# CMU-SAFARI/Scrooge

Hardware: AMD Instinct MI355X
Metric: aligned pairs/s (+ GCUPS) at W=64, 10kb reads; 1/2/4/8 MI355X (higher is better)
Workload: dtype u64

## Files before the change

scrooge_amd/api.py:

```python
import contextlib
import ctypes as C
import os
import subprocess
import sys
from collections import namedtuple

HERE = os.path.dirname(os.path.abspath(__file__))
_LIB = None

Alignment = namedtuple("Alignment", ["cigar", "edit_distance"])

SCRG_OK = 0
SCRG_ERR_INVALID_ARG = 1
SCRG_ERR_BAD_BASE = 2
SCRG_ERR_NO_DEVICE = 3
SCRG_ERR_HIP = 4
SCRG_ERR_OOM = 5
SCRG_ERR_CIGAR_OVERFLOW = 6
SCRG_PAIR_OVER_EDIT_LIMIT = 7
SCRG_PAIR_NOT_BEST = 8
SCRG_OUT_ALL, SCRG_OUT_TEXT, SCRG_OUT_RUNS = 0, 1, 2
SCRG_OUT_BEST = 4
SCRG_OUT_DISTANCE = 16
DEVICE_STATUS_OVER_EDIT_LIMIT = 2
# ... 896 lines not shown
        with self._call_limit(max_edits, max_edit_per_mille):
            self._check(self.lib.scrg_align_device(self.h, C.byref(self._params(kw)), int(n_pairs),
                                                   _ptr(seq), _ptr(pairs), _ptr(runs), _ptr(ed),
                                                   _ptr(n_runs), _ptr(status)))

    def align_device_edits(self, n_pairs, seq, pairs, streams_u8, ed, stream_len, status, n_runs=None, max_edits=None,
                           max_edit_per_mille=None, **kw):
        with self._call_limit(max_edits, max_edit_per_mille):
            self._check(self.lib.scrg_align_device_edits(self.h, C.byref(self._params(kw)), int(n_pairs),
                                                         _ptr(seq), _ptr(pairs), _ptr(streams_u8), _ptr(ed),
                                                         _ptr(stream_len), _ptr(status), _ptr(n_runs)))

    def align_device_distance(self, n_pairs, seq, pairs, ed, text_end, status, max_edits=None, max_edit_per_mille=None, **kw):
        with self._call_limit(max_edits, max_edit_per_mille):
            self._check(_lazy(self.lib, "scrg_align_device_distance")(self.h, C.byref(self._params(kw)), int(n_pairs), _ptr(seq), _ptr(pairs),
                                                                      _ptr(ed), _ptr(text_end), _ptr(status)))

    def diff_lengths(self, kind, n_pairs, seq, pairs, runs, run_offset, run_offset_stride, n_runs, diff_len, **kw):
        ro = C.c_void_p(pairs.data_ptr() + 32) if run_offset is None else _ptr(run_offset)
        self._check(_lazy(self.lib, "scrg_diff_lengths")(self.h, C.byref(self._params(kw)), _diff_kind(kind), int(n_pairs), _ptr(seq), _ptr(pairs),
                                                         _ptr(runs), ro, int(run_offset_stride), _ptr(n_runs), _ptr(diff_len)))

    def diff_render(self, kind, n_pairs, seq, pairs, runs, run_offset, run_offset_stride, n_runs, diff_len, diff_offset, diff_text_u8, bad_i32,
                    capacity=None, **kw):
        ro = C.c_void_p(pairs.data_ptr() + 32) if run_offset is None else _ptr(run_offset)
        cap = int(diff_text_u8.numel()) if capacity is None else int(capacity)
        self._check(_lazy(self.lib, "scrg_diff_render")(self.h, C.byref(self._params(kw)), _diff_kind(kind), int(n_pairs), _ptr(seq), _ptr(pairs),
                                                        _ptr(runs), ro, int(run_offset_stride), _ptr(n_runs), _ptr(diff_len), _ptr(diff_offset),
                                                        _ptr(diff_text_u8), cap, _ptr(bad_i32)))

    def compact_runs(self, n_pairs, pairs, runs, n_runs, dense_off, dense):
        self._check(self.lib.scrg_compact_runs(self.h, int(n_pairs), _ptr(pairs), _ptr(runs),
                                               _ptr(n_runs), _ptr(dense_off), _ptr(dense)))

    def select_best(self, n_pairs, group_key_u32, ed, status, n_runs, is_best_u8=None):
        self._check(_lazy(self.lib, "scrg_select_best")(self.h, int(n_pairs), _ptr(group_key_u32), _ptr(ed), _ptr(status), _ptr(n_runs),
                                                        _ptr(is_best_u8)))

    def compact_runs_packed(self, n_pairs, pairs, runs, n_runs, dense_off, packed_u8, **kw):
        self._check(self.lib.scrg_compact_runs_packed(self.h, C.byref(self._params(kw)), int(n_pairs), _ptr(pairs),
                                                      _ptr(runs), _ptr(n_runs), _ptr(dense_off), _ptr(packed_u8)))

    def unpack_runs(self, n_runs, packed_u8, runs_u8):
        self._check(self.lib.scrg_unpack_runs(self.h, int(n_runs), _ptr(packed_u8), _ptr(runs_u8)))

    def encode_edit_stream(self, n_pairs, pairs, runs, n_runs, stream_u8, stream_off_i64, stream_len_i32, total_i64, **kw):
        self._check(self.lib.scrg_encode_edit_stream(self.h, C.byref(self._params(kw)), int(n_pairs), _ptr(pairs), _ptr(runs), _ptr(n_runs),
                                                     _ptr(stream_u8), int(stream_u8.numel()), _ptr(stream_off_i64),
                                                     _ptr(stream_len_i32), _ptr(total_i64)))

    def decode_edit_stream(self, n_pairs, stream_u8, stream_off_i64, stream_len_i32, read_len_i64, read_len_stride,
                           dense_off_i64, dense_u8, n_runs_i32, bad_i32, **kw):
        self._check(self.lib.scrg_decode_edit_stream(self.h, C.byref(self._params(kw)), int(n_pairs), _ptr(stream_u8),
                                                     int(stream_u8.numel()), _ptr(stream_off_i64), _ptr(stream_len_i32), _ptr(read_len_i64),
                                                     int(read_len_stride),
                                                     _ptr(dense_off_i64) if dense_off_i64 is not None else None,
                                                     _ptr(dense_u8) if dense_u8 is not None else None,
                                                     int(dense_u8.numel() * dense_u8.element_size() // 2) if dense_u8 is not None else 0,
                                                     _ptr(n_runs_i32), _ptr(bad_i32)))

    def ascii_to_twobit(self, count, lens, ascii_off, ascii, twobit_off, twobit, bad):
        self._check(self.lib.scrg_ascii_to_twobit(self.h, int(count), _ptr(lens), _ptr(ascii_off),
                                                  _ptr(ascii), _ptr(twobit_off), _ptr(twobit),
                                                  _ptr(bad)))

    def last_kernel_ms(self):
        ms = C.c_float(0)
        self._check(self.lib.scrg_last_kernel_ms(self.h, C.byref(ms)))
        return float(ms.value)

    def debug_stats(self):
        out = (C.c_uint64 * 12)()
        self._check(self.lib.scrg_debug_stats(self.h, out))
        return {"rounds": int(out[0]), "dc_steps": int(out[1]), "tb_macro_steps": int(out[2]),
                "cycles_fetch": int(out[3]), "cycles_setup": int(out[4]), "cycles_dc": int(out[5]),
                "cycles_tb": int(out[6]), "cycles_tb_loop": int(out[7]), "diag_rounds": int(out[8]),
                "diag_fallbacks": int(out[9]), "cycles_diag_dc": int(out[10]), "cycles_diag_tb": int(out[11])}

    def debug_stats_lane(self):
        out = (C.c_uint64 * 12)()
        self._check(self.lib.scrg_debug_stats(self.h, out))
        o = [int(x) for x in out]
        big = 1 << 62
        return {"rounds": o[0], "short_text_rounds": o[1], "cycles_pass1": o[2], "cycles_fetch": o[3], "cycles_setup": o[4],
                "cycles_table": o[5], "cycles_traceback": o[6], "life_ticks_sum": o[7], "last_start": o[8],
                "first_start": big - o[9], "last_end": o[10], "first_end": big - o[11]}

    def resolved_params(self, **kw):
        out = Params()
        st = self.lib.scrg_params_resolve(C.byref(self._params(kw)), C.byref(out))
        if st != SCRG_OK:
            raise ScroogeError(st, "invalid parameters")
        return out

    def query_launch(self, **kw):
        a, b, c, d = C.c_int32(), C.c_int32(), C.c_int32(), C.c_int32()
        self._check(self.lib.scrg_query_launch(self.h, C.byref(self._params(kw)), C.byref(a),
                                               C.byref(b), C.byref(c), C.byref(d)))
        return {"n_waves": a.value, "pairs_per_wave": b.value, "lds_bytes": c.value,
                "n_cus": d.value}
```

scrooge_amd/csrc/genasm_kernels.h:

```cpp
#pragma once

#include <hip/hip_runtime.h>
#include <stdint.h>

#include <type_traits>

#include "../../include/scrooge_amd.h"

namespace scrg {

constexpr int SPILL_ROWS = 72;

struct AlignArgs {
    const uint64_t* seq;
    const scrg_pair_desc* pairs;
    uint16_t* runs;
    int64_t* ed;
    union {
        uint32_t* n_runs;
        uint32_t* text_end;
    };
    uint32_t* status;
    uint32_t* run_count;
    uint32_t* counter;
    uint32_t* spill;
    uint32_t n_pairs;
    int32_t W;
    int32_t tb_limit;
    int32_t lds_rows;
    uint32_t text_stride;
    uint32_t read_stride;
    uint64_t* stats;
    int32_t debug;
    uint32_t stranded;
    uint32_t max_edits;
    uint32_t per_mille;
    uint32_t text_rev;
};
enum LaneOutput : int { LANE_OUT_RUNS = 0, LANE_OUT_EDITS = 1, LANE_OUT_NONE = 2 };
template <typename F> inline void with_lane_output(LaneOutput out, F&& f)
{
    if (out == LANE_OUT_NONE) f(std::integral_constant<int, LANE_OUT_NONE>{});
    else if (out == LANE_OUT_EDITS) f(std::integral_constant<int, LANE_OUT_EDITS>{});
    else f(std::integral_constant<int, LANE_OUT_RUNS>{});
}
enum LaneStatus : uint32_t { LANE_STATUS_DONE = 0, LANE_STATUS_OVERFLOW = 1, LANE_STATUS_OVER_EDIT_LIMIT = 2, LANE_STATUS_NOT_BEST = 3 };

#if defined(SCRG_ABLATE) && !defined(SCRG_STATS)
#define SCRG_STATS 1
#endif
#if defined(SCRG_STATS) && !defined(SCRG_SELECT)
#define SCRG_SELECT 1
#endif
constexpr int32_t SCRG_SWITCH_NO_DIAG = 32;
constexpr int32_t SCRG_SWITCH_MW_TABLE = 256;
constexpr int32_t SCRG_SWITCH_SPLIT = 512;
constexpr int32_t SCRG_SWITCH_NO_SPLIT = 1024;
constexpr int32_t SCRG_SAFE_SWITCHES = SCRG_SWITCH_NO_DIAG | SCRG_SWITCH_MW_TABLE | SCRG_SWITCH_SPLIT | SCRG_SWITCH_NO_SPLIT;
#ifdef SCRG_SELECT
#define SCRG_SEL(flags, bit) (((flags) & (bit)) != 0)
constexpr bool SCRG_HAVE_SELECT = true;
#else
#define SCRG_SEL(flags, bit) false
constexpr bool SCRG_HAVE_SELECT = false;
#endif
#ifdef SCRG_STATS
#define SCRG_TIMING(args) ((args).stats != nullptr)
#define SCRG_SW(args, bit) (((args).debug & (bit)) != 0)
constexpr bool SCRG_HAVE_STATS = true;
#else
#define SCRG_TIMING(args) false
#define SCRG_SW(args, bit) false
constexpr bool SCRG_HAVE_STATS = false;
#endif
#ifdef SCRG_ABLATE
#define SCRG_ABL(args, bit) (((args).debug & (bit)) != 0)
constexpr int32_t SCRG_ALLOWED_SWITCHES = 0x1ff | SCRG_SAFE_SWITCHES;
#elif defined(SCRG_STATS)
#define SCRG_ABL(args, bit) false
constexpr int32_t SCRG_ALLOWED_SWITCHES = SCRG_SAFE_SWITCHES | 1 | 64 | 128;
#elif defined(SCRG_SELECT)
#define SCRG_ABL(args, bit) false
constexpr int32_t SCRG_ALLOWED_SWITCHES = SCRG_SAFE_SWITCHES;
#else
#define SCRG_ABL(args, bit) false
constexpr int32_t SCRG_ALLOWED_SWITCHES = 0;
#endif

#ifdef __HIPCC__
#define SCRG_HD __host__ __device__
#else
#define SCRG_HD
#endif

hipError_t launch_align(int lanes_per_pair, const AlignArgs& a, int grid, size_t lds_bytes, hipStream_t s);
hipError_t launch_align_multiword(int lanes_per_pair, const AlignArgs& a, int grid, size_t lds_bytes, hipStream_t s);
hipError_t launch_align_lane(const AlignArgs& a, int grid, size_t lds_bytes, hipStream_t s, LaneOutput out = LANE_OUT_RUNS);
SCRG_HD inline unsigned lane_lds_bytes(LaneOutput out = LANE_OUT_RUNS) { return 64u * ((out == LANE_OUT_NONE ? 0u : 68u + 36u) + 32u + 8u); }
hipError_t launch_align_lane_split(const AlignArgs& a, int grid, hipStream_t s);
constexpr int LANE_SPLIT_PRODUCERS_PER_CU = 8;

SCRG_HD inline unsigned lane_mw_len_bytes(int tb_limit) { return (((unsigned)tb_limit + 3u) & ~3u) + 4u; }
SCRG_HD inline unsigned lane_mw_lds_bytes(int tb_limit, LaneOutput out = LANE_OUT_RUNS) { return out == LANE_OUT_NONE ? 0u : 64u * (68u + lane_mw_len_bytes(tb_limit)); }
SCRG_HD inline size_t lane_mw_table_bytes(int tb_limit) { return (size_t)tb_limit * 2u * ((unsigned)tb_limit / 64u + 1u) * 64u * 8u; }
hipError_t launch_align_lane_mw(const AlignArgs& a, int grid, size_t lds_bytes, hipStream_t s, LaneOutput out = LANE_OUT_RUNS);
SCRG_HD inline bool lane_wide_serves(int W, int tb_limit) { return W <= 128 && tb_limit >= 32 && tb_limit <= 63; }
SCRG_HD inline unsigned lane_wide_lds_bytes(int W, LaneOutput out = LANE_OUT_RUNS) { return 64u * ((out == LANE_OUT_NONE ? 0u : 68u + 36u) + (W <= 64 ? 40u : 80u)); }
hipError_t launch_align_lane_wide(const AlignArgs& a, int grid, size_t lds_bytes, hipStream_t s, LaneOutput out = LANE_OUT_RUNS);
SCRG_HD inline bool lane_parts_serves(int W, int tb_limit)
{
    return W > 64 && W <= 256 && ((tb_limit >= 64 && tb_limit <= 127) || (W > 128 && tb_limit >= 1 && tb_limit <= 63));
}
SCRG_HD inline unsigned lane_parts_lds_bytes(int W, LaneOutput out = LANE_OUT_RUNS)
{
    const unsigned nw = ((unsigned)W + 63u) / 64u, slot = nw == 2u ? 16u : 32u;
    return 64u * ((out == LANE_OUT_NONE ? 0u : 68u + 20u) + 5u * slot + 16u * nw);
}
SCRG_HD inline size_t lane_parts_checkpoint_bytes(int W) { return (size_t)8u * 4u * (((unsigned)W + 63u) / 64u) * 64u * 4u; }
hipError_t launch_align_lane_parts(const AlignArgs& a, int grid, size_t lds_bytes, hipStream_t s, LaneOutput out = LANE_OUT_RUNS);

SCRG_HD inline unsigned stored_row_dwords(int W, int tb_limit)
{
    if (W <= 64) return tb_limit > 31 ? 128u : 32u;
    const unsigned sw = (unsigned)tb_limit / 64u + 1u;
    return 64u * sw * sw * 2u;
}

constexpr unsigned DIAG_WIDE_ROWS = 8;
constexpr unsigned DIAG_LATE_BASE = 128;
constexpr unsigned DIAG_PARK_DWORD = 392;
constexpr unsigned DIAG_SLOT_DWORDS = DIAG_PARK_DWORD + 4 + 1;
SCRG_HD inline unsigned slot_stride_dwords(int W, int tb_limit, int lanes_per_pair, int lds_rows)
{
    unsigned s = (unsigned)lds_rows * stored_row_dwords(W, tb_limit) + 1u;
    if (W == 64 && lanes_per_pair == 8 && tb_limit <= 31 && s < DIAG_SLOT_DWORDS) s = DIAG_SLOT_DWORDS;
    return s;
}

enum AlignForm : int {
    FORM_ROWS,
    FORM_ROWS_MW,
// ... 72 lines not shown
```

scrooge_amd/csrc/genasm_lane_kernel.hip:

```cpp

#include <hip/hip_runtime.h>
#include <stdint.h>
#include <type_traits>

#include "lane_common.h"

namespace scrg {

constexpr int LANE_TB_COLS = 31;
constexpr uint32_t LANE_RING_BYTES = 68;
constexpr uint32_t LANE_SCRATCH_BYTES = 36;
constexpr uint32_t LANE_EQ_BYTES = 32;
constexpr uint32_t LANE_NOMATCH_BYTES = 8;
constexpr uint32_t LANE_WAVE_LDS_BYTES = 64u * (LANE_RING_BYTES + LANE_SCRATCH_BYTES + LANE_EQ_BYTES + LANE_NOMATCH_BYTES);
constexpr uint32_t LANE_EQ_SLOT_STRIDE = 512;
constexpr uint32_t LANE_EQ_REGION_BYTES = 4u * LANE_EQ_SLOT_STRIDE;
constexpr uint32_t LANE_EQ_FIELD_MASK = 3u * LANE_EQ_SLOT_STRIDE;
constexpr uint32_t LANE_REST_BYTES = LANE_WAVE_LDS_BYTES - LANE_EQ_REGION_BYTES;
constexpr int LANE_EQ_AHEAD = 8;

__device__ __forceinline__ uint32_t lane_read_offset(uint32_t fwd_offset, uint32_t read_idx, uint32_t read_len, uint32_t revm)
{
    return bitop3<TT_BFI>(sub_sat_u32(read_len - read_idx, 64u), fwd_offset, revm);
}
__device__ __forceinline__ void lane_pattern_rev(const Planes pw, uint32_t left, uint32_t revm, bool any_rev, uint64_t& rlo, uint64_t& rhi)
{
    rlo = brev64(pw.lo);
    rhi = brev64(pw.hi);
    if (any_rev) {
        const uint32_t sh = sub_sat_u32(64u, left);
        const uint64_t flo = ~(pw.lo << sh), fhi = ~(pw.hi << sh);
        rlo = ((uint64_t)bitop3<TT_BFI>((uint32_t)(flo >> 32), (uint32_t)(rlo >> 32), revm) << 32) | bitop3<TT_BFI>((uint32_t)flo, (uint32_t)rlo, revm);
        rhi = ((uint64_t)bitop3<TT_BFI>((uint32_t)(fhi >> 32), (uint32_t)(rhi >> 32), revm) << 32) | bitop3<TT_BFI>((uint32_t)fhi, (uint32_t)rhi, revm);
    }
}

constexpr uint32_t LANE_TEXT_REV = 1u << 7;
__device__ __forceinline__ uint32_t lane_text_offset(uint32_t ref_idx, uint32_t text_len, uint32_t tr_in)
{
    return bitop3<TT_BFI>(text_rev_at(text_len, ref_idx, 0u).at, ref_idx, neg_mask(tr_in << 24));
}
__device__ __forceinline__ void lane_text_rev(Planes& tw, uint32_t text_len, uint32_t ref_idx, uint32_t tr_in)
{
    const uint32_t tm = neg_mask(tr_in << 24);
    const uint32_t sh = text_rev_at(text_len, ref_idx, 0u).sh;
    const uint64_t flo = ~brev64(tw.lo << sh), fhi = ~brev64(tw.hi << sh);
    tw.lo = ((uint64_t)bitop3<TT_BFI>((uint32_t)(flo >> 32), (uint32_t)(tw.lo >> 32), tm) << 32) | bitop3<TT_BFI>((uint32_t)flo, (uint32_t)tw.lo, tm);
    tw.hi = ((uint64_t)bitop3<TT_BFI>((uint32_t)(fhi >> 32), (uint32_t)(tw.hi >> 32), tm) << 32) | bitop3<TT_BFI>((uint32_t)fhi, (uint32_t)tw.hi, tm);
}

template <bool SHORT_N>
__device__ __forceinline__ void lane_window_table(const Planes tw, const uint64_t rlo, const uint64_t rhi, const uint32_t n, const uint32_t m,
                                                  const uint32_t stop, uint64_t (&tab)[LANE_TB_COLS],
                                                  const uint32_t eq_b, const uint32_t nomatch_b)
{
    const uint64_t valid = ~0ull << (64u - m);
    const uint32_t rl0 = (uint32_t)rlo, rl1 = (uint32_t)(rlo >> 32), rh0 = (uint32_t)rhi, rh1 = (uint32_t)(rhi >> 32);
    const uint32_t iv0 = ~(uint32_t)valid, iv1 = ~(uint32_t)(valid >> 32);
    {
        lds_write64(eq_b, make_uint2(~(rl0 | rh0) | iv0, ~(rl1 | rh1) | iv1));
        lds_write64(eq_b + LANE_EQ_SLOT_STRIDE, make_uint2((rl0 & ~rh0) | iv0, (rl1 & ~rh1) | iv1));
        lds_write64(eq_b + 2u * LANE_EQ_SLOT_STRIDE, make_uint2((~rl0 & rh0) | iv0, (~rl1 & rh1) | iv1));
        lds_write64(eq_b + 3u * LANE_EQ_SLOT_STRIDE, make_uint2((rl0 & rh0) | iv0, (rl1 & rh1) | iv1));
        if (SHORT_N) lds_write64(nomatch_b, make_uint2(iv0, iv1));
    }
    const uint32_t tl0 = (uint32_t)tw.lo, tl1 = (uint32_t)(tw.lo >> 32), th0 = (uint32_t)tw.hi, th1 = (uint32_t)(tw.hi >> 32);
    const uint32_t xe0 = bitop3<TT_BFI>(tl0, th0 << 1, 0x55555555u), xo0 = bitop3<TT_BFI>(th0, tl0 >> 1, 0xaaaaaaaau);
    const uint32_t xe1 = bitop3<TT_BFI>(tl1, th1 << 1, 0x55555555u), xo1 = bitop3<TT_BFI>(th1, tl1 >> 1, 0xaaaaaaaau);
    auto eq_addr = [&](int i) -> uint32_t {
        const int b = i & 31;
        const uint32_t x = (b & 1) ? (i < 32 ? xo0 : xo1) : (i < 32 ? xe0 : xe1);
        const int f = (b & 1) ? b - 1 : b;
        const uint32_t u = f >= 9 ? x >> (f - 9) : x << (9 - f);
        const uint32_t a = bitop3<TT_ANDOR>(u, LANE_EQ_FIELD_MASK, eq_b);
        if (!SHORT_N) return a;
        return bitop3<TT_BFI>(a, nomatch_b, neg_mask((uint32_t)i - n));
    };
    uint2 eqw[LANE_EQ_AHEAD];
#pragma unroll
    for (int k = 0; k < LANE_EQ_AHEAD; k++) eqw[k] = lds_read64(eq_addr(63 - k));
    uint32_t pv0 = (uint32_t)valid, pv1 = (uint32_t)(valid >> 32), mv0 = 0u, mv1 = 0u;
#pragma unroll
    for (int i = 63; i >= 0; i--) {
        const uint2 eq_now = eqw[(63 - i) % LANE_EQ_AHEAD];
        if (i - LANE_EQ_AHEAD >= 0) eqw[(63 - i) % LANE_EQ_AHEAD] = lds_read64(eq_addr(i - LANE_EQ_AHEAD));
        {
            const uint32_t eq0 = eq_now.x, eq1 = eq_now.y;
            const uint32_t xv0 = eq0 | mv0, xv1 = eq1 | mv1;
            const uint32_t t0 = eq0 & pv0, t1 = eq1 & pv1;
            const uint64_t sum = add64(((uint64_t)t1 << 32) | t0, ((uint64_t)pv1 << 32) | pv0);
            const uint32_t xh0 = bitop3<TT_XH>((uint32_t)sum, pv0, eq0), xh1 = bitop3<TT_XH>((uint32_t)(sum >> 32), pv1, eq1);
            const uint32_t ph0 = bitop3<TT_PH>(mv0, xh0, pv0), ph1 = bitop3<TT_PH>(mv1, xh1, pv1);
            const uint32_t mh0 = pv0 & xh0, mh1 = pv1 & xh1;
            const uint64_t phs = shl1(((uint64_t)ph1 << 32) | ph0);
            const uint64_t mhs = shl1(((uint64_t)mh1 << 32) | mh0);
            pv0 = bitop3<TT_PVN>((uint32_t)mhs, xv0, (uint32_t)phs);
            pv1 = bitop3<TT_PVN>((uint32_t)(mhs >> 32), xv1, (uint32_t)(phs >> 32));
            mv0 = (uint32_t)phs & xv0;
            mv1 = (uint32_t)(phs >> 32) & xv1;
            if (i < LANE_TB_COLS)
                tab[i] = ((uint64_t)bitop3<TT_NOR3>(pv1, ph1, stop) << 32) | bitop3<TT_V0>(pv1, ph1, xh1);
        }
    }
}

template <int OUT>
__global__ __launch_bounds__(256, 4) void genasm_lane_kernel(AlignArgs a)
{
    constexpr bool EDITS = OUT == LANE_OUT_EDITS, NONE = OUT == LANE_OUT_NONE;
    constexpr uint32_t REST_BYTES = NONE ? 64u * LANE_NOMATCH_BYTES : LANE_REST_BYTES;
    constexpr uint32_t STAGE_BYTES = NONE ? 0u : 64u * (LANE_RING_BYTES + LANE_SCRATCH_BYTES);
    extern __shared__ __attribute__((aligned(16))) uint32_t lds[];
    char* const lds_b = reinterpret_cast<char*>(lds);

    const uint32_t lane = threadIdx.x & 63u;
    const uint32_t wave = threadIdx.x >> 6, wpg = blockDim.x >> 6;
    const uint32_t wave_b = wpg * LANE_EQ_REGION_BYTES + wave * REST_BYTES;
    const uint32_t ring_b = wave_b + lane * LANE_RING_BYTES;
    const uint32_t scr_b = wave_b + 64u * LANE_RING_BYTES + lane * LANE_SCRATCH_BYTES;
    uint8_t* const lds8 = reinterpret_cast<uint8_t*>(lds);
    const uint32_t lds0 = (uint32_t)(uintptr_t)(__attribute__((address_space(3))) char*)lds_b;
    const uint32_t eq_b = lds0 + wave * LANE_EQ_REGION_BYTES + lane * 8u;
    const uint32_t nomatch_b = lds0 + wave_b + STAGE_BYTES + lane * LANE_NOMATCH_BYTES;
    const uint32_t W = (uint32_t)a.W;
    const uint32_t TBL = (uint32_t)a.tb_limit;

    bool has_pair = false;
    uint32_t pair = 0;
    const uint64_t* text_w = a.seq;
    const uint64_t* read_w = a.seq;
    uint32_t tr_in = 0;
    uint64_t cigar_off = 0;
    uint32_t text_len = 0, read_len = 0, cigar_cap = 0;
    uint32_t ref_idx = 0, read_idx = 0, edits = 0;
    uint32_t lim = 0xffffffffu;
    uint32_t revm = 0;
    int32_t nr = -1;
    uint32_t flushed = 0;
    uint32_t pos = 0;
    uint32_t mbase = 0;
    WindowWords twords = {0, 0, 0, 0}, pwords = {0, 0, 0, 0};
    bool queue_empty = false;
    const bool timing = SCRG_TIMING(a);
    uint64_t cy_fetch = 0, cy_setup = 0, cy_dc = 0, cy_tb = 0, cy_p1 = 0;
    uint32_t st_rounds = 0, st_gen = 0;
    const uint64_t rt0 = timing ? __builtin_amdgcn_s_memrealtime() : 0;

    auto write_piece = [&]() {
        if constexpr (!NONE) scrg::write_piece<EDITS>(a, lds, ring_b, cigar_off, cigar_cap, flushed, !SCRG_ABL(a, 16));
    };
    auto flush_pieces = [&]() {
        if constexpr (!NONE) {
            const bool need = has_pair && (EDITS ? pos - flushed >= 32u : nr - (int32_t)flushed >= 15);
            if (__any(need)) {
                if (need) write_piece();
            }
        }
    };
    auto ring_guard = [&](uint32_t fill, uint32_t limit) {
        if (__any(has_pair && fill >= limit)) {
            if (has_pair && fill >= (EDITS ? 32u : 16u)) write_piece();
        }
    };

    uint32_t rot = hw_wave_slot();
    for (;;) {
        if (!SCRG_SW(a, 1)) rotate_priority(rot++);
        const uint64_t tm0 = timing ? __builtin_readcyclecounter() : 0;
        for (;;) {
            const bool over = has_pair && edits > lim;
            const bool fin = over || (has_pair && read_idx >= read_len);
            if (__any(fin)) {
                if (over) abandon_pair<OUT>(a, pair, edits);
                else if constexpr (NONE) { if (fin) retire_pair_distance(a, pair, edits, ref_idx); }
                else if (fin) retire_pair<EDITS>(a, lds, ring_b, pair, cigar_off, cigar_cap, flushed, EDITS ? pos : (uint32_t)(nr + 1), nr, edits, !SCRG_ABL(a, 16));
                has_pair = has_pair && !fin;
            }
            const bool want = !has_pair && !queue_empty;
            if (!__any(want)) break;
            const uint32_t idx = claim_pairs(a, lane, want);
            const bool got = want && idx < a.n_pairs;
            if (__any(want && idx >= a.n_pairs)) queue_empty = true;
            if (got) {
                const scrg_pair_desc pd = a.pairs[idx];
                pair = idx;
                const TextStretch ts = text_stretch(pd.text_off, pd.text_len, a.text_rev != 0u, a.text_stride);
                text_w = a.seq + (ts.off >> 5);
                const uint64_t r_off = a.stranded ? pd.read_off & ~SCRG_READ_REVCOMP : pd.read_off;
                revm = (a.stranded && (pd.read_off & SCRG_READ_REVCOMP)) ? 0xffffffffu : 0u;
                read_w = a.seq + (r_off >> 5);
                tr_in = ((uint32_t)ts.off & 31u) | (((uint32_t)r_off & 31u) << 8) | (ts.rev ? LANE_TEXT_REV : 0u);
                text_len = ts.len;
                read_len = (uint32_t)pd.read_len;
                lim = pair_edit_limit(a, read_len);
                if constexpr (NONE) {
                    ref_idx = read_idx = edits = 0;
                } else {
                    cigar_off = pd.cigar_off;
                    cigar_cap = pd.cigar_cap > 0xffffffffull ? 0xffffffffu : (uint32_t)pd.cigar_cap;
                    ref_idx = read_idx = edits = flushed = pos = mbase = 0;
                    nr = -1;
                }
                has_pair = true;
                twords = load_window_words_at(text_w, tr_in & 31u, ts.rev ? text_rev_at(text_len, 0u, 0u).at : 0u, a.text_stride);
                pwords = load_window_words_at(read_w, tr_in >> 8, lane_read_offset(0u, 0u, read_len, revm), a.read_stride);
            }
        }
        if (!__any(has_pair)) break;
        const bool wave_rev = a.stranded && __any(has_pair && revm != 0u);
        const bool wave_trev = a.text_rev && __any(has_pair && (tr_in & LANE_TEXT_REV) != 0u);

        const uint64_t tm1 = timing ? __builtin_readcyclecounter() : 0;
        const uint32_t n = has_pair ? min(W, sub_sat_u32(text_len, ref_idx)) : 0u;
        const uint32_t m = has_pair ? min(W, read_len - read_idx) : 1u;
        Planes tw = window_planes(twords);
        const Planes pw = window_planes(pwords);
        if (wave_trev) lane_text_rev(tw, text_len, ref_idx, tr_in);
        asm volatile("" :: "v"(tw.lo), "v"(tw.hi), "v"(pw.lo), "v"(pw.hi) : "memory");
        flush_pieces();
        const uint64_t tm2 = timing ? __builtin_readcyclecounter() : 0;

        uint64_t tab[LANE_TB_COLS];
        const uint32_t jlim = has_pair ? min(m, TBL) : 0u;
        const uint32_t stop = 0x80000000u >> jlim;
        const bool short_n = __any(has_pair && n != 64u);
        uint64_t rlo, rhi;
        lane_pattern_rev(pw, read_len - read_idx, revm, wave_rev, rlo, rhi);
        if (SCRG_ABL(a, 2)) {
#pragma unroll
            for (int i = 0; i < LANE_TB_COLS; i++) tab[i] = ((uint64_t)~stop << 32) | (((uint32_t)tw.lo * (uint32_t)(i + 1)) | stop);
        } else if (short_n) {
            lane_window_table<true>(tw, rlo, rhi, n, m, stop, tab, eq_b, nomatch_b);
            st_gen++;
        } else {
            lane_window_table<false>(tw, rlo, rhi, n, m, stop, tab, eq_b, nomatch_b);
        }
        const uint64_t tm3 = timing ? __builtin_readcyclecounter() : 0;

        {
            uint32_t j = 0, ti, nDm = 0, Xm = 0, nIm = 0;
            auto walk = [&](auto full_tag) {
                constexpr bool FULL = decltype(full_tag)::value;
#pragma unroll
                for (int i = 0; i < LANE_TB_COLS; i++) {
                    if (!FULL && (uint32_t)i >= TBL) continue;
                    const uint32_t x = bitop3<TT_NIV>((uint32_t)(tab[i] >> 32), (uint32_t)tab[i], stop) << j;
                    const uint32_t ni = ffbh_u32(x);
                    if constexpr (!NONE) lds8[scr_b + i] = (uint8_t)ni;
                    nIm = __builtin_amdgcn_alignbit(nIm, x, 31);
                    j += ni;
                    const uint64_t both = tab[i] << j;
                    const uint32_t nt1 = (uint32_t)(both >> 32), t0 = (uint32_t)both;
                    nDm = __builtin_amdgcn_alignbit(nDm, nt1, 31);
                    Xm = __builtin_amdgcn_alignbit(Xm, t0, 31);
                    j -= neg_mask(nt1);
                }
            };
            if (SCRG_ABL(a, 8)) { j = jlim; nDm = ~0u; }
            else if (TBL == (uint32_t)LANE_TB_COLS) walk(std::true_type{});
            else walk(std::false_type{});
            if (timing) cy_p1 += __builtin_readcyclecounter() - tm3;
            const uint32_t TBc = min(TBL, (uint32_t)LANE_TB_COLS);
            const uint32_t nsh = 32u - TBc;
            const uint32_t notD = nDm << nsh, Xraw = Xm << nsh;
            const uint32_t Draw = ~notD;
            const uint32_t Im = ~nIm << nsh;
            const uint32_t ti_stopped = (31u - ffbl_u32((notD >> 1) | Im)) & 31u;
            ti = bitop3<TT_BFI>(TBc, ti_stopped, neg_mask(j - jlim));
            const uint32_t A = ~(0xffffffffu >> ti);
            const uint32_t D = Draw & A, X = Xraw & A;
            const uint32_t B = ((D ^ (D >> 1)) | (X ^ (X >> 1)) | Im | 0x80000000u) & A;
            const uint32_t nD = (uint32_t)__builtin_popcount(D), nX = (uint32_t)__builtin_popcount(X);
            edits += j - ti + 2u * nD + nX;
            ref_idx += ti;
            read_idx += j;
            twords = load_window_words_at(text_w, tr_in & 31u, wave_trev ? lane_text_offset(ref_idx, text_len, tr_in) : ref_idx, a.text_stride);
            const uint32_t left_x = read_idx ^ read_len;
            const uint32_t fwd_at = read_idx & neg_mask(left_x | (0u - left_x));
            pwords = load_window_words_at(read_w, tr_in >> 8, wave_rev ? lane_read_offset(fwd_at, read_idx, read_len, revm) : fwd_at, a.read_stride);

            if constexpr (NONE) {
                (void)B;
            } else if constexpr (EDITS) {
                uint32_t E = SCRG_ABL(a, 4) ? 0u : (D | X | Im);
                nr += (int32_t)(__builtin_popcount(B) + __builtin_popcount(Im));
                uint32_t c = ffbh_u32(E);
                uint32_t ni = lds8[scr_b + c];
                auto put = [&](uint32_t at, uint32_t b) { lds8[ring_b + (at & 63u)] = (uint8_t)b; };
                auto event = [&]() {
                    const uint32_t sh = 31u - c;
                    const uint32_t bit = 0x80000000u >> (c & 31u);
                    uint32_t iB = __builtin_amdgcn_ubfe(Im, sh, 1), dx = __builtin_amdgcn_ubfe(D | X, sh, 1);
                    const uint32_t xB = __builtin_amdgcn_ubfe(X, sh, 1);
                    const uint32_t t = mbase + c;
                    E = bitop3<TT_ANDN>(E, bit, bit);
                    const uint32_t nx = ffbh_u32(E);
                    const uint32_t step = 0xC0u - 0x80u * xB;
                    const bool side = ni * iB > 3u;
                    if (__any(side)) {
                        if (side) {
                            auto emit = [&](uint32_t b) {
                                put(pos, b);
                                pos++;
                                if (pos - flushed >= 32u) write_piece();
                            };
                            emit(0x80u | t);
                            for (uint32_t q = 1; q < ni; q++) emit(0x80u);
                            mbase = 0u - c;
                            if (dx) {
                                emit(step);
                                mbase = ~c;
                            }
                            iB = dx = 0;
                        }
                    }
                    put(pos, 0x80u | t);
                    put(pos + 1u, 0x80u);
                    put(pos + 2u, 0x80u);
                    pos += iB ? ni : 0u;
                    put(pos, step | (iB ? 0u : t));
                    pos += dx;
                    mbase = dx ? ~c : (iB ? 0u - c : mbase);
                    ni = lds8[scr_b + nx];
                    c = nx;
                };
                uint32_t trips = 0;
                while (__any(E != 0u)) {
                    if (trips >= 2u) ring_guard(pos - flushed, 50u);
                    event();
                    event();
                    trips++;
                }
                put(pos, mbase + ti);
                pos += has_pair ? 1u : 0u;
                mbase = 0;
            } else {
            uint32_t E = SCRG_ABL(a, 4) ? 0u : (B | Im);
            uint32_t c0 = ffbh_u32(E);
            E = bitop3<TT_ANDN>(E, 0x80000000u >> (c0 & 31u), 0u);
            uint32_t c1 = ffbh_u32(E);
            uint32_t q = 2u * (uint32_t)nr + 2u;
            auto event = [&](uint32_t& c, const uint32_t ni, const uint32_t nx) {
                const uint32_t sh = 31u - c;
                const uint32_t aI = ring_b + (q & 62u);
                q = add_twice(q, __builtin_amdgcn_ubfe(Im, sh, 1));
                const uint32_t w = add3(mad24(__builtin_amdgcn_ubfe(X, sh, 1), 27u << 8, mad24(__builtin_amdgcn_ubfe(D, sh, 1), 7u << 8, sh)),
                                        min(nx, ti), ((uint32_t)'=' << 8) - 31u);
                const uint32_t aS = ring_b + (q & 62u);
                q = add_twice(q, __builtin_amdgcn_ubfe(B, sh, 1));
                E = bitop3<TT_ANDN>(E, 0x80000000u >> (nx & 31u), 0u);
                c = ffbh_u32(E);
                *reinterpret_cast<uint16_t*>(lds_b + aI) = (uint16_t)(((uint32_t)'I' << 8) | ni);
                *reinterpret_cast<uint16_t*>(lds_b + aS) = (uint16_t)w;
            };
            uint32_t trips = 0;
            while (__any(c0 < 32u)) {
                const uint32_t n0 = lds8[scr_b + c0], n1 = lds8[scr_b + c1];
                if (trips >= 4u) ring_guard((q >> 1) - flushed, 27u);
                event(c0, n0, c1);
                event(c1, n1, c0);
                trips++;
            }
            nr = ((int32_t)q >> 1) - 1;
            }
        }
        st_rounds++;
        if (timing) {
            const uint64_t tm4 = __builtin_readcyclecounter();
            cy_fetch += tm1 - tm0;
            cy_setup += tm2 - tm1;
            cy_dc += tm3 - tm2;
            cy_tb += tm4 - tm3;
        }
    }
    if (timing && lane == 0) {
        atomicAdd((unsigned long long*)&a.stats[0], (unsigned long long)st_rounds);
        atomicAdd((unsigned long long*)&a.stats[1], (unsigned long long)st_gen);
        atomicAdd((unsigned long long*)&a.stats[2], (unsigned long long)cy_p1);
        atomicAdd((unsigned long long*)&a.stats[3], (unsigned long long)cy_fetch);
        atomicAdd((unsigned long long*)&a.stats[4], (unsigned long long)cy_setup);
        atomicAdd((unsigned long long*)&a.stats[5], (unsigned long long)cy_dc);
        atomicAdd((unsigned long long*)&a.stats[6], (unsigned long long)cy_tb);
        const uint64_t rt1 = __builtin_amdgcn_s_memrealtime();
        atomicAdd((unsigned long long*)&a.stats[7], (unsigned long long)(rt1 - rt0));
        atomicMax((unsigned long long*)&a.stats[8], (unsigned long long)rt0);
        atomicMax((unsigned long long*)&a.stats[9], (unsigned long long)((1ull << 62) - rt0));
        atomicMax((unsigned long long*)&a.stats[10], (unsigned long long)rt1);
        atomicMax((unsigned long long*)&a.stats[11], (unsigned long long)((1ull << 62) - rt1));
    }
}

constexpr uint32_t SPLIT_FIELDS = 6;
constexpr uint32_t SPLIT_BUF_BYTES = SPLIT_FIELDS * 256u + 64u * LANE_SCRATCH_BYTES;
constexpr uint32_t SPLIT_PAIR_LDS_BYTES = 64u * (LANE_RING_BYTES + LANE_EQ_BYTES + LANE_NOMATCH_BYTES) + 2u * SPLIT_BUF_BYTES;
constexpr uint32_t SPLIT_WG_LDS_BYTES = 4u * SPLIT_PAIR_LDS_BYTES + 64u;
constexpr uint32_t SPLIT_VALID = 1u << 8, SPLIT_FIRST = 1u << 9, SPLIT_LAST = 1u << 10;
constexpr uint32_t SPLIT_OVER = 1u << 11;

__global__ __launch_bounds__(512, 2) void genasm_lane_split_kernel(AlignArgs a)
{
    extern __shared__ __attribute__((aligned(16))) uint32_t lds[];
    char* const lds_b = reinterpret_cast<char*>(lds);
    uint8_t* const lds8 = reinterpret_cast<uint8_t*>(lds);
    const uint32_t lane = threadIdx.x & 63u;
    const uint32_t wave = threadIdx.x >> 6, duo = wave & 3u;
    const bool consumer = wave >= 4u;
    const uint32_t duo_b = 4u * LANE_EQ_REGION_BYTES + duo * (SPLIT_PAIR_LDS_BYTES - LANE_EQ_REGION_BYTES);
    const uint32_t ring_b = duo_b + lane * LANE_RING_BYTES;
    const uint32_t lds0 = (uint32_t)(uintptr_t)(__attribute__((address_space(3))) char*)lds_b;
    const uint32_t eq_b = lds0 + duo * LANE_EQ_REGION_BYTES + lane * 8u;
    const uint32_t nomatch_b = lds0 + duo_b + 64u * LANE_RING_BYTES + lane * LANE_NOMATCH_BYTES;
    const uint32_t bufs_b = duo_b + 64u * (LANE_RING_BYTES + LANE_NOMATCH_BYTES);
    const uint32_t flags_w = (4u * SPLIT_PAIR_LDS_BYTES) >> 2;
    const uint32_t W = (uint32_t)a.W;
    const uint32_t TBL = (uint32_t)a.tb_limit;
    const uint32_t TBc = min(TBL, (uint32_t)LANE_TB_COLS);
    const uint32_t nsh = 32u - TBc;
    auto rec_w = [&](uint32_t buf, uint32_t field) -> uint32_t { return ((bufs_b + buf * SPLIT_BUF_BYTES) >> 2) + field * 64u + lane; };
    auto len_b = [&](uint32_t buf) -> uint32_t { return bufs_b + buf * SPLIT_BUF_BYTES + SPLIT_FIELDS * 256u + lane * LANE_SCRATCH_BYTES; };
    auto all_done = [&](uint32_t r) -> bool {
        const uint32_t f = flags_w + (r & 1u) * 4u;
        return (lds[f] & lds[f + 1] & lds[f + 2] & lds[f + 3]) != 0u;
    };

    if (!consumer) {
        bool has_pair = false, active = true;
        uint32_t pair = 0;
        uint64_t text_off = 0, read_off = 0;
        uint32_t text_len = 0, read_len = 0;
        uint32_t ref_idx = 0, read_idx = 0, edits = 0;
        uint32_t lim = 0xffffffffu;
        uint32_t revm = 0;
        bool trev = false;
        WindowWords twords = {0, 0, 0, 0}, pwords = {0, 0, 0, 0};
        bool queue_empty = false;
        uint32_t st_rounds = 0;
        const uint32_t slot = hw_wave_slot();
        for (uint32_t r = 0;; r++) {
            const uint32_t buf = r & 1u;
            uint32_t first = 0;
            if (active) {
                if (!SCRG_SW(a, 1)) rotate_priority(r + slot);
                has_pair = has_pair && read_idx < read_len && edits <= lim;
                for (;;) {
                    const bool want = !has_pair && !queue_empty;
                    if (!__any(want)) break;
                    const uint32_t idx = claim_pairs(a, lane, want);
                    const bool got = want && idx < a.n_pairs;
                    if (__any(want && idx >= a.n_pairs)) queue_empty = true;
                    if (got) {
                        const LanePair p = unpack_pair(a, idx);
                        pair = idx;
                        text_off = p.text_off;
                        read_off = p.read_off;
                        revm = p.rev ? 0xffffffffu : 0u;
                        trev = p.trev;
                        text_len = p.text_len;
                        read_len = p.read_len;
                        lim = pair_edit_limit(a, p.read_len);
                        ref_idx = read_idx = edits = 0;
// ... 188 lines not shown
```

Before: 65.24 million.

## Add banded 32-bit bit-vector window table with adaptive fallback to full table

Adds a banded variant of the per-window DP table that tracks a 32-cell diagonal band in 32-bit words instead of the full 64-bit columns, then walks the traceback on that band. If any lane's window distance exceeds a safe threshold, the wave recomputes the full table, reusing the already written Eq masks. A per-wave controller backs off from trying the band for a growing number of rounds after repeated failures. It is meant to cut ALU work in the table-build step when windows have few edits, at the cost of wasted band work and divergence on high-error windows.

```diff
diff --git a/scrooge_amd/api.py b/scrooge_amd/api.py
--- a/scrooge_amd/api.py
+++ b/scrooge_amd/api.py
@@ -1002,7 +1002,9 @@
         self._check(self.lib.scrg_debug_stats(self.h, out))
         o = [int(x) for x in out]
         big = 1 << 62
-        return {"rounds": o[0], "short_text_rounds": o[1], "cycles_pass1": o[2], "cycles_fetch": o[3], "cycles_setup": o[4],
+        m21 = (1 << 21) - 1
+        return {"rounds": o[0] & 0xffffffff, "band_backed_off_rounds": o[0] >> 32, "short_text_rounds": o[1] & m21,
+                "band_rounds": (o[1] >> 21) & m21, "band_redone_rounds": o[1] >> 42, "cycles_pass1": o[2], "cycles_fetch": o[3], "cycles_setup": o[4],
                 "cycles_table": o[5], "cycles_traceback": o[6], "life_ticks_sum": o[7], "last_start": o[8],
                 "first_start": big - o[9], "last_end": o[10], "first_end": big - o[11]}
 
diff --git a/scrooge_amd/csrc/genasm_kernels.h b/scrooge_amd/csrc/genasm_kernels.h
--- a/scrooge_amd/csrc/genasm_kernels.h
+++ b/scrooge_amd/csrc/genasm_kernels.h
@@ -56,7 +56,9 @@
 constexpr int32_t SCRG_SWITCH_MW_TABLE = 256;
 constexpr int32_t SCRG_SWITCH_SPLIT = 512;
 constexpr int32_t SCRG_SWITCH_NO_SPLIT = 1024;
-constexpr int32_t SCRG_SAFE_SWITCHES = SCRG_SWITCH_NO_DIAG | SCRG_SWITCH_MW_TABLE | SCRG_SWITCH_SPLIT | SCRG_SWITCH_NO_SPLIT;
+constexpr int32_t SCRG_SWITCH_NO_BAND = 4096;
+constexpr int32_t SCRG_SWITCH_BAND_ALWAYS = 8192;
+constexpr int32_t SCRG_SAFE_SWITCHES = SCRG_SWITCH_NO_DIAG | SCRG_SWITCH_MW_TABLE | SCRG_SWITCH_SPLIT | SCRG_SWITCH_NO_SPLIT | SCRG_SWITCH_NO_BAND | SCRG_SWITCH_BAND_ALWAYS;
 #ifdef SCRG_SELECT
 #define SCRG_SEL(flags, bit) (((flags) & (bit)) != 0)
 constexpr bool SCRG_HAVE_SELECT = true;
diff --git a/scrooge_amd/csrc/genasm_lane_kernel.hip b/scrooge_amd/csrc/genasm_lane_kernel.hip
--- a/scrooge_amd/csrc/genasm_lane_kernel.hip
+++ b/scrooge_amd/csrc/genasm_lane_kernel.hip
@@ -49,30 +49,46 @@
     tw.hi = ((uint64_t)bitop3<TT_BFI>((uint32_t)(fhi >> 32), (uint32_t)(tw.hi >> 32), tm) << 32) | bitop3<TT_BFI>((uint32_t)fhi, (uint32_t)tw.hi, tm);
 }
 
-template <bool SHORT_N>
-__device__ __forceinline__ void lane_window_table(const Planes tw, const uint64_t rlo, const uint64_t rhi, const uint32_t n, const uint32_t m,
-                                                  const uint32_t stop, uint64_t (&tab)[LANE_TB_COLS],
-                                                  const uint32_t eq_b, const uint32_t nomatch_b)
-{
-    const uint64_t valid = ~0ull << (64u - m);
+template <bool NOMATCH>
+__device__ __forceinline__ void lane_write_eq(const uint64_t rlo, const uint64_t rhi, const uint32_t iv0, const uint32_t iv1,
+                                              const uint32_t eq_b, const uint32_t nomatch_b)
+{
     const uint32_t rl0 = (uint32_t)rlo, rl1 = (uint32_t)(rlo >> 32), rh0 = (uint32_t)rhi, rh1 = (uint32_t)(rhi >> 32);
-    const uint32_t iv0 = ~(uint32_t)valid, iv1 = ~(uint32_t)(valid >> 32);
+    lds_write64(eq_b, make_uint2(~(rl0 | rh0) | iv0, ~(rl1 | rh1) | iv1));
+    lds_write64(eq_b + LANE_EQ_SLOT_STRIDE, make_uint2((rl0 & ~rh0) | iv0, (rl1 & ~rh1) | iv1));
+    lds_write64(eq_b + 2u * LANE_EQ_SLOT_STRIDE, make_uint2((~rl0 & rh0) | iv0, (~rl1 & rh1) | iv1));
+    lds_write64(eq_b + 3u * LANE_EQ_SLOT_STRIDE, make_uint2((rl0 & rh0) | iv0, (rl1 & rh1) | iv1));
+    if (NOMATCH) lds_write64(nomatch_b, make_uint2(iv0, iv1));
+}
+struct LaneEqAddr {
+    uint32_t xe0, xo0, xe1, xo1, eq_b;
+    __device__ __forceinline__ LaneEqAddr(const Planes tw, const uint32_t eq_b_) : eq_b(eq_b_)
     {
-        lds_write64(eq_b, make_uint2(~(rl0 | rh0) | iv0, ~(rl1 | rh1) | iv1));
-        lds_write64(eq_b + LANE_EQ_SLOT_STRIDE, make_uint2((rl0 & ~rh0) | iv0, (rl1 & ~rh1) | iv1));
-        lds_write64(eq_b + 2u * LANE_EQ_SLOT_STRIDE, make_uint2((~rl0 & rh0) | iv0, (~rl1 & rh1) | iv1));
-        lds_write64(eq_b + 3u * LANE_EQ_SLOT_STRIDE, make_uint2((rl0 & rh0) | iv0, (rl1 & rh1) | iv1));
-        if (SHORT_N) lds_write64(nomatch_b, make_uint2(iv0, iv1));
-    }
-    const uint32_t tl0 = (uint32_t)tw.lo, tl1 = (uint32_t)(tw.lo >> 32), th0 = (uint32_t)tw.hi, th1 = (uint32_t)(tw.hi >> 32);
-    const uint32_t xe0 = bitop3<TT_BFI>(tl0, th0 << 1, 0x55555555u), xo0 = bitop3<TT_BFI>(th0, tl0 >> 1, 0xaaaaaaaau);
-    const uint32_t xe1 = bitop3<TT_BFI>(tl1, th1 << 1, 0x55555555u), xo1 = bitop3<TT_BFI>(th1, tl1 >> 1, 0xaaaaaaaau);
-    auto eq_addr = [&](int i) -> uint32_t {
+        const uint32_t tl0 = (uint32_t)tw.lo, tl1 = (uint32_t)(tw.lo >> 32), th0 = (uint32_t)tw.hi, th1 = (uint32_t)(tw.hi >> 32);
+        xe0 = bitop3<TT_BFI>(tl0, th0 << 1, 0x55555555u), xo0 = bitop3<TT_BFI>(th0, tl0 >> 1, 0xaaaaaaaau);
+        xe1 = bitop3<TT_BFI>(tl1, th1 << 1, 0x55555555u), xo1 = bitop3<TT_BFI>(th1, tl1 >> 1, 0xaaaaaaaau);
+    }
+    __device__ __forceinline__ uint32_t at(const int i) const
+    {
         const int b = i & 31;
         const uint32_t x = (b & 1) ? (i < 32 ? xo0 : xo1) : (i < 32 ? xe0 : xe1);
         const int f = (b & 1) ? b - 1 : b;
         const uint32_t u = f >= 9 ? x >> (f - 9) : x << (9 - f);
-        const uint32_t a = bitop3<TT_ANDOR>(u, LANE_EQ_FIELD_MASK, eq_b);
+        return bitop3<TT_ANDOR>(u, LANE_EQ_FIELD_MASK, eq_b);
+    }
+};
+
+template <bool SHORT_N>
+__device__ __forceinline__ void lane_window_table(const Planes tw, const uint64_t rlo, const uint64_t rhi, const uint32_t n, const uint32_t m,
+                                                  const uint32_t stop, uint64_t (&tab)[LANE_TB_COLS],
+                                                  const uint32_t eq_b, const uint32_t nomatch_b, const bool write_eq = true)
+{
+    const uint64_t valid = ~0ull << (64u - m);
+    const uint32_t iv0 = ~(uint32_t)valid, iv1 = ~(uint32_t)(valid >> 32);
+    if (write_eq) lane_write_eq<SHORT_N>(rlo, rhi, iv0, iv1, eq_b, nomatch_b);
+    const LaneEqAddr ea(tw, eq_b);
+    auto eq_addr = [&](int i) -> uint32_t {
+        const uint32_t a = ea.at(i);
         if (!SHORT_N) return a;
         return bitop3<TT_BFI>(a, nomatch_b, neg_mask((uint32_t)i - n));
     };
@@ -104,10 +120,74 @@
     }
 }
 
+constexpr int BAND_UP = 10, BAND_DOWN = 21, BAND_SAFE = 19;
+static_assert(BAND_UP + BAND_DOWN + 1 == 32 && BAND_SAFE / 2 + 1 <= BAND_UP && BAND_SAFE + 1 <= BAND_DOWN, "the band holds every cell a safe walk asks about");
+constexpr int TT_D0 = bitop3_table([](int sum, int pv, int xv) { return (sum ^ pv) | xv; });
+constexpr int TT_OR3 = bitop3_table([](int a, int b, int c) { return a | b | c; });
+constexpr int TT_NIV_BAND = bitop3_table([](int v1, int v0, int stop) { return ~(v1 & v0) | stop; });
+__device__ __forceinline__ uint64_t lane_band_stop0(const uint32_t TBL)
+{
+    uint64_t s0 = 0x8000000000000000ull >> (TBL + (uint32_t)BAND_UP);
+    asm volatile("" : "+s"(s0));
+    return s0;
+}
+__device__ __forceinline__ uint32_t lane_band_stop(const uint64_t stop0, const int i)
+{
+    return (uint32_t)((stop0 << i) >> 32);
+}
+constexpr bool LANE_BAND_TABLE = true;
+constexpr uint32_t BAND_STRETCH = 32, BAND_REDO_MAX = 6;
+__device__ __forceinline__ uint32_t add_masked(uint32_t acc, const uint32_t x, const uint32_t mask)
+{
+    uint32_t t;
+    asm volatile("v_and_b32 %0, %2, %3\n\tv_add_u32 %1, %1, %0" : "=&v"(t), "+v"(acc) : "s"(mask), "v"(x));
+    return acc;
+}
+__device__ __forceinline__ uint32_t lane_window_table_band(const Planes tw, const uint64_t rlo, const uint64_t rhi, const uint32_t TBL,
+                                                           uint64_t (&tab)[LANE_TB_COLS], const uint32_t eq_b)
+{
+    lane_write_eq<false>(rlo, rhi, 0u, 0u, eq_b, 0u);
+    const LaneEqAddr ea(tw, eq_b);
+    const uint64_t stop0 = lane_band_stop0(TBL);
+    auto band_eq = [&](const uint2 w, const int i) -> uint32_t {
+        const int s = 62 - i - BAND_DOWN;
+        if (s >= 32) return w.y >> (s - 32);
+        if (s > 0) return __builtin_amdgcn_alignbit(w.y, w.x, (uint32_t)s);
+        if (s == 0) return w.x;
+        return __builtin_amdgcn_alignbit(w.x, 0xffffffffu, (uint32_t)(32 + s));
+    };
+    uint2 eqw[LANE_EQ_AHEAD];
+#pragma unroll
+    for (int k = 0; k < LANE_EQ_AHEAD; k++) eqw[k] = lds_read64(ea.at(63 - k));
+    uint32_t pv = ~0u << (BAND_DOWN + 1), mv = 0u;
+    uint32_t fd = 0u;
+#pragma unroll
+    for (int i = 63; i >= 0; i--) {
+        const uint32_t eq = band_eq(eqw[(63 - i) % LANE_EQ_AHEAD], i);
+        if (i - LANE_EQ_AHEAD >= 0) eqw[(63 - i) % LANE_EQ_AHEAD] = lds_read64(ea.at(i - LANE_EQ_AHEAD));
+        const uint32_t xv = eq | mv;
+        const uint32_t d0 = bitop3<TT_D0>((eq & pv) + pv, pv, xv);
+        const uint32_t ph = bitop3<TT_PH>(mv, d0, pv);
+        const uint32_t mh = pv & d0;
+        fd = add_masked(fd, d0, 1u << (32 - BAND_UP));
+        const uint32_t xvs = xv >> 1;
+        pv = bitop3<TT_PVN>(mh, xvs, ph);
+        mv = ph & xvs;
+        if (i < LANE_TB_COLS) {
+            const uint32_t phs = ph >> 1;
+            uint32_t v1 = bitop3<TT_OR3>(pv, phs, lane_band_stop(stop0, i)), v0 = bitop3<TT_V0>(pv, phs, d0 >> 1);
+            asm volatile("" : "+v"(v1), "+v"(v0));
+            tab[i] = ((uint64_t)v1 << 32) | v0;
+        }
+    }
+    return 64u - (fd >> (32 - BAND_UP));
+}
+
 template <int OUT>
 __global__ __launch_bounds__(256, 4) void genasm_lane_kernel(AlignArgs a)
 {
     constexpr bool EDITS = OUT == LANE_OUT_EDITS, NONE = OUT == LANE_OUT_NONE;
+    constexpr bool BAND = LANE_BAND_TABLE;
     constexpr uint32_t REST_BYTES = NONE ? 64u * LANE_NOMATCH_BYTES : LANE_REST_BYTES;
     constexpr uint32_t STAGE_BYTES = NONE ? 0u : 64u * (LANE_RING_BYTES + LANE_SCRATCH_BYTES);
     extern __shared__ __attribute__((aligned(16))) uint32_t lds[];
@@ -144,6 +224,8 @@
     const bool timing = SCRG_TIMING(a);
     uint64_t cy_fetch = 0, cy_setup = 0, cy_dc = 0, cy_tb = 0, cy_p1 = 0;
     uint32_t st_rounds = 0, st_gen = 0;
+    uint32_t band_ctl = 0;
+    uint32_t st_band = 0, st_redone = 0, st_skipped = 0;
     const uint64_t rt0 = timing ? __builtin_amdgcn_s_memrealtime() : 0;
 
     auto write_piece = [&]() {
@@ -226,39 +308,76 @@
         const bool short_n = __any(has_pair && n != 64u);
         uint64_t rlo, rhi;
         lane_pattern_rev(pw, read_len - read_idx, revm, wave_rev, rlo, rhi);
-        if (SCRG_ABL(a, 2)) {
+        uint32_t j = 0, ti, nDm = 0, Xm = 0, nIm = 0;
+        auto walk = [&](auto full_tag, auto band_tag) {
+            constexpr bool FULL = decltype(full_tag)::value;
+            constexpr bool BANDED = decltype(band_tag)::value;
+            const uint64_t stop0 = BANDED ? lane_band_stop0(TBL) : 0ull;
 #pragma unroll
-            for (int i = 0; i < LANE_TB_COLS; i++) tab[i] = ((uint64_t)~stop << 32) | (((uint32_t)tw.lo * (uint32_t)(i + 1)) | stop);
-        } else if (short_n) {
-            lane_window_table<true>(tw, rlo, rhi, n, m, stop, tab, eq_b, nomatch_b);
-            st_gen++;
-        } else {
-            lane_window_table<false>(tw, rlo, rhi, n, m, stop, tab, eq_b, nomatch_b);
-        }
-        const uint64_t tm3 = timing ? __builtin_readcyclecounter() : 0;
-
+            for (int i = 0; i < LANE_TB_COLS; i++) {
+                if (!FULL && (uint32_t)i >= TBL) continue;
+                const uint32_t x = (BANDED ? bitop3<TT_NIV_BAND>((uint32_t)(tab[i] >> 32), (uint32_t)tab[i], lane_band_stop(stop0, i))
+                                           : bitop3<TT_NIV>((uint32_t)(tab[i] >> 32), (uint32_t)tab[i], stop)) << j;
+                const uint32_t ni = ffbh_u32(x);
+                if constexpr (!NONE) lds8[scr_b + i] = (uint8_t)ni;
+                nIm = __builtin_amdgcn_alignbit(nIm, x, 31);
+                j += ni;
+                const uint64_t both = tab[i] << j;
+                const uint32_t nt1 = (uint32_t)(both >> 32), t0 = (uint32_t)both;
+                nDm = __builtin_amdgcn_alignbit(nDm, nt1, 31);
+                Xm = __builtin_amdgcn_alignbit(Xm, t0, 31);
+                if (BANDED) j += neg_mask(nt1);
+                else j -= neg_mask(nt1);
+            }
+        };
+        bool walked = false, eq_written = false;
+        uint64_t tm3 = 0;
+        if constexpr (BAND) {
+            if (W == 64u && !short_n && !__any(has_pair && m != 64u) && !SCRG_SEL(a.debug, SCRG_SWITCH_NO_BAND) && !SCRG_ABL(a, 2) && !SCRG_ABL(a, 8)) {
+                if ((band_ctl >> 16) != 0u) {
+                    band_ctl -= 1u << 16;
+                    st_skipped++;
+                } else {
+                    const uint32_t d_band = lane_window_table_band(tw, rlo, rhi, TBL, tab, eq_b);
+                    walked = !__any(has_pair && d_band > (uint32_t)BAND_SAFE);
+                    eq_written = true;
+                    st_band++;
+                    st_redone += walked ? 0u : 1u;
+                    band_ctl += walked ? 1u : 0x101u;
+                    if (((band_ctl >> 8) & 15u) > BAND_REDO_MAX && !SCRG_SEL(a.debug, SCRG_SWITCH_BAND_ALWAYS)) {
+                        const uint32_t fails = (band_ctl >> 12) & 15u;
+                        band_ctl = (32u << (16u + fails)) | (min(fails + 1u, 6u) << 12);
+                    } else if ((band_ctl & 255u) == BAND_STRETCH) {
+                        band_ctl = 0u;
+                    }
+                    if (walked) {
+                        tm3 = timing ? __builtin_readcyclecounter() : 0;
+                        j = (uint32_t)BAND_UP;
+                        if (TBL == (uint32_t)LANE_TB_COLS) walk(std::true_type{}, std::true_type{});
+                        else walk(std::false_type{}, std::true_type{});
+                        j = has_pair ? j + TBL - (uint32_t)BAND_UP : 0u;
+                        nDm = has_pair ? ~nDm : 0u;
+                        nIm = has_pair ? nIm : ~0u;
+                    }
+                }
+            }
+        }
+        if (!walked) {
+            if (SCRG_ABL(a, 2)) {
+#pragma unroll
+                for (int i = 0; i < LANE_TB_COLS; i++) tab[i] = ((uint64_t)~stop << 32) | (((uint32_t)tw.lo * (uint32_t)(i + 1)) | stop);
+            } else if (short_n) {
+                lane_window_table<true>(tw, rlo, rhi, n, m, stop, tab, eq_b, nomatch_b);
+                st_gen++;
+            } else {
+                lane_window_table<false>(tw, rlo, rhi, n, m, stop, tab, eq_b, nomatch_b, !eq_written);
+            }
+            tm3 = timing ? __builtin_readcyclecounter() : 0;
+            if (SCRG_ABL(a, 8)) { j = jlim; nDm = ~0u; }
+            else if (TBL == (uint32_t)LANE_TB_COLS) walk(std::true_type{}, std::false_type{});
+            else walk(std::false_type{}, std::false_type{});
+        }
         {
-            uint32_t j = 0, ti, nDm = 0, Xm = 0, nIm = 0;
-            auto walk = [&](auto full_tag) {
-                constexpr bool FULL = decltype(full_tag)::value;
-#pragma unroll
-                for (int i = 0; i < LANE_TB_COLS; i++) {
-                    if (!FULL && (uint32_t)i >= TBL) continue;
-                    const uint32_t x = bitop3<TT_NIV>((uint32_t)(tab[i] >> 32), (uint32_t)tab[i], stop) << j;
-                    const uint32_t ni = ffbh_u32(x);
-                    if constexpr (!NONE) lds8[scr_b + i] = (uint8_t)ni;
-                    nIm = __builtin_amdgcn_alignbit(nIm, x, 31);
-                    j += ni;
-                    const uint64_t both = tab[i] << j;
-                    const uint32_t nt1 = (uint32_t)(both >> 32), t0 = (uint32_t)both;
-                    nDm = __builtin_amdgcn_alignbit(nDm, nt1, 31);
-                    Xm = __builtin_amdgcn_alignbit(Xm, t0, 31);
-                    j -= neg_mask(nt1);
-                }
-            };
-            if (SCRG_ABL(a, 8)) { j = jlim; nDm = ~0u; }
-            else if (TBL == (uint32_t)LANE_TB_COLS) walk(std::true_type{});
-            else walk(std::false_type{});
             if (timing) cy_p1 += __builtin_readcyclecounter() - tm3;
             const uint32_t TBc = min(TBL, (uint32_t)LANE_TB_COLS);
             const uint32_t nsh = 32u - TBc;
@@ -374,8 +493,8 @@
         }
     }
     if (timing && lane == 0) {
-        atomicAdd((unsigned long long*)&a.stats[0], (unsigned long long)st_rounds);
-        atomicAdd((unsigned long long*)&a.stats[1], (unsigned long long)st_gen);
+        atomicAdd((unsigned long long*)&a.stats[0], (unsigned long long)st_rounds | ((unsigned long long)st_skipped << 32));
+        atomicAdd((unsigned long long*)&a.stats[1], (unsigned long long)st_gen | ((unsigned long long)st_band << 21) | ((unsigned long long)st_redone << 42));
         atomicAdd((unsigned long long*)&a.stats[2], (unsigned long long)cy_p1);
         atomicAdd((unsigned long long*)&a.stats[3], (unsigned long long)cy_fetch);
         atomicAdd((unsigned long long*)&a.stats[4], (unsigned long long)cy_setup);
```

Result: faster. 75.89 million (median of 6 runs) (+16.3%).
